# NingZhang1/pyscf_isdf

Measured on AMD Instinct MI355X. Metric: isdf_build_plus_get_jk_wall_time, lower is better.
Workload: dtype f64

## Files before the change

### include/mi355_isdf.h

```cpp
#ifndef MI355_ISDF_H
#define MI355_ISDF_H

#include <stdint.h>

#ifdef __cplusplus
extern "C" {
#endif

typedef struct isdf_ctx* isdf_handle;

#define ISDF_OK 0
#define ISDF_ERR_ARG 1
#define ISDF_ERR_HIP 2
#define ISDF_ERR_LIB 3
#define ISDF_ERR_NUM 4

int isdf_abi_version(void);

int isdf_create(int device_id, isdf_handle* out);
int isdf_destroy(isdf_handle h);
int isdf_set_stream(isdf_handle h, void* hip_stream);
const char* isdf_last_error(isdf_handle h);
int64_t isdf_workspace_bytes(isdf_handle h);
int isdf_release_workspace(isdf_handle h);
// ... 44 lines not shown
                   int nblk, const int64_t* blk_off, const int32_t* nip,
                   double tol, double tie_rtol,
                   double* d_L, int64_t ldL, int64_t* d_piv, int32_t* rank);

int isdf_select_ip_ws(isdf_handle h, const double* d_ao, int nao, int64_t ld,
                      int nblk, const int64_t* blk_off, const int32_t* nip,
                      double tol, double tie_rtol,
                      double* d_L, int64_t ldL, int64_t* d_piv, int32_t* rank,
                      void* d_work, int64_t work_bytes);
int64_t isdf_select_ip_work_bytes(int nao, int64_t m);

int isdf_select_ip_gram(isdf_handle h, double* d_A, int m, int64_t ldA, int nip, double tol, double tie_rtol,
                        int panel, int64_t* d_piv, int32_t* rank);

int isdf_select_ip_cplx(isdf_handle h, const double* d_ao, int nao, int nh, int64_t ld,
                        int nblk, const int64_t* blk_off, const int32_t* nip,
                        double tol, double tie_rtol,
                        double* d_L, int64_t ldL, int64_t* d_piv, int32_t* rank);

int isdf_fit_from_chol(isdf_handle h, double* d_L, int k, int64_t m, int64_t ldL,
                       const int64_t* d_piv);

int isdf_fit_prepare(isdf_handle h, const double* d_ao, int nao, int64_t ld,
                     const int64_t* d_ip, int P, double reg_rel, double* d_aoP, double* d_chol,
                     double* reg_used);
int isdf_fit_apply(isdf_handle h, const double* d_chol, const double* d_aoP, int P, int nao,
                   const double* d_ao, int64_t ng, int64_t ld, int forward_only,
                   double* d_theta, int64_t ldt);
int isdf_fit_prepare_cplx(isdf_handle h, const double* d_ao, int nao, int nh, int64_t ld,
                          const int64_t* d_ip, int P, double reg_rel, double* d_aoP, double* d_chol,
                          double* reg_used);
int isdf_fit_apply_cplx(isdf_handle h, const double* d_chol, const double* d_aoP, int P, int nao, int nh,
                        const double* d_ao, int64_t ng, int64_t ld, int forward_only,
                        double* d_theta, int64_t ldt);
int isdf_fit_global(isdf_handle h, const double* d_ao, int nao, int64_t ngrids, int64_t ld,
                    const int64_t* d_ip, int P, double reg_rel, double* d_theta, int64_t ldt,
                    double* d_aoP, double* reg_used);

int isdf_gather_aoP(isdf_handle h, const double* d_ao, int nao, int64_t ld, const int64_t* d_ip, int P,
                    double* d_aoP);
int isdf_gram_sq(isdf_handle h, const double* d_aoP, int P, int nao, int nh, double* d_A);
int isdf_pair_gram_rows(isdf_handle h, const double* d_aoP, int P, int nao, int nh, const double* d_ao,
                        int64_t ng, int64_t ld, double* d_B, int64_t ldb);
int isdf_block_chol(isdf_handle h, const double* d_A, int P, int nblk, const int32_t* blk_off,
                    double shift_rel, double* d_D, double* shift_used);
int isdf_block_solve(isdf_handle h, const double* d_D, int P, int nblk, const int32_t* blk_off, int side,
                     int trans, double* d_X, int64_t n, int64_t ldx);
int isdf_block_invert(isdf_handle h, const double* d_D, int P, int nblk, const int32_t* blk_off, double* d_Dinv);
int isdf_block_apply(isdf_handle h, const double* d_Dinv, int64_t ldd, int nblk, const int32_t* blk_off,
                     double* d_X, int64_t n, int64_t ldx);
int isdf_pair_rows_block_apply(isdf_handle h, const double* d_aoP, int P, int nao, const double* d_ao, int64_t ng,
                               int64_t ld, const double* d_Dinv, int64_t ldd, int nblk, const int32_t* blk_off,
                               double* d_B, int64_t ldb);

int isdf_gram_prod(isdf_handle h, const double* d_aoP, int P, int nao, const double* d_psiP, int nocc, double* d_A);
int isdf_pair_prod_rows(isdf_handle h, const double* d_aoP, int P, int nao, const double* d_psiP, int nocc,
                        const double* d_ao, int64_t ld, const double* d_psi, int64_t ldpsi, int64_t ng,
                        double* d_B, int64_t ldb);
int isdf_factor_solve_half(isdf_handle h, const double* d_fac, int P, int backward, double* d_X, int64_t n, int64_t ldx);
int isdf_gram_prod_cplx(isdf_handle h, const double* d_aoP, int P, int nao, int nh, const double* d_psiP, int npsi, int npsi_h,
                        double* d_A);
int isdf_pair_prod_rows_cplx(isdf_handle h, const double* d_aoP, int P, int nao, int nh, const double* d_psiP, int npsi,
                             int npsi_h, const double* d_ao, int64_t ld, const double* d_psi, int64_t ldpsi, int64_t ng,
                             double* d_B, int64_t ldb);

int isdf_shift_diag(isdf_handle h, double* d_A, int P, double shift_rel);
int isdf_chol_inplace(isdf_handle h, double* d_A, int P, double shift_rel, double* d_scratch, double* reg_used);

int isdf_factor_solve(isdf_handle h, const double* d_fac, int P, double* d_X, int64_t n, int64_t ldx);

int isdf_bj_probe_vectors(isdf_handle h, double* d_T, int n, const double* d_fac, const double* d_D, int P,
                          int nblk, const int32_t* blk_off);
int isdf_rows_combine(isdf_handle h, const double* d_E, int n, int64_t ldE, int rows, const double* d_Y,
                      int64_t ng, int64_t ldy, double* d_F, int64_t ldf, int accumulate);

int isdf_bj_probe_rows(isdf_handle h, double* d_T, int n, const double* d_fac, const double* d_D, int P, int nblk,
                       const int32_t* blk_off, const double* d_Yp, int64_t ng, int64_t ldy, double* d_F, int64_t ldf);

int isdf_gather_T(isdf_handle h, const double* d_L, int k, int64_t ldL, const int64_t* d_piv,
                  double* d_T);
int isdf_W_from_factor(isdf_handle h, const double* d_F, int P, int kind, double* d_M, int64_t ldm);

int isdf_coulomb_W(isdf_handle h, const double* d_theta, int P, int64_t ldt,
                   const int32_t mesh[3], const double a[9],
                   int row0, int nrows, int batch, int upper_only, double* d_W, int64_t ldw);
int isdf_coulG_half(isdf_handle h, const int32_t mesh[3], const double a[9], double* d_out);
int isdf_spectral_supported(isdf_handle h, const int32_t mesh[3], int batch, int* ok);
int isdf_spectral_rows(isdf_handle h, const double* d_in, int nrows, int64_t ld, const int32_t mesh[3], const int32_t* d_idx,
                       const double* d_scale, int npts, int batch, double* d_out, int64_t ldx);
int isdf_coulomb_rows(isdf_handle h, const double* d_in, int nrows, int64_t ld,
                      const int32_t mesh[3], const double a[9], int batch, double* d_out, int64_t ldo);
int isdf_symmetrize_upper(isdf_handle h, double* d_W, int P, int64_t ldw);
int isdf_symmetrize_mean(isdf_handle h, double* d_W, int P, int64_t ldw, int antisymmetric);

int isdf_get_j(isdf_handle h, const double* d_ao, int nao, int64_t ngrids, int64_t ld,
               const int32_t mesh[3], const double a[9],
               const double* d_dm, int nset, double* d_vj);
int isdf_rho(isdf_handle h, const double* d_ao, int nao, int64_t ng, int64_t ld,
             const double* d_dm, int nset, double* d_rho, int64_t ldrho);
int isdf_coulomb_potential(isdf_handle h, double* d_rho_inout, int nset, int64_t ldrho,
                           const int32_t mesh[3], const double a[9]);
int isdf_vj_from_vR(isdf_handle h, const double* d_ao, int nao, int64_t ng, int64_t ld,
                    const double* d_vR, int nset, int64_t ldv, double* d_vj);

int isdf_get_k_exact(isdf_handle h, const double* d_ao, int nao, int64_t ngrids, int64_t ld,
                     const double* d_C, int nocc, const int32_t mesh[3], const double a[9],
// ... 84 lines not shown
```

### pyscf_isdf_amd/backend.py

```python
import ctypes
import os
import numpy as np
import torch
from . import lib as _lib

_vp = ctypes.c_void_p


def _np_ptr(a):
    return a.ctypes.data_as(_vp)


class HipBackend:
    name = 'hip-gfx950'

    def __init__(self, device=0):
        if not torch.cuda.is_available():
            raise _lib.IsdfError('no GPU visible to torch; the ISDF path has no CPU fallback')
        self.device = torch.device('cuda', device)
        torch.cuda.set_device(self.device)
        self.handle = _lib.Handle(device)
        if os.environ.get('ISDF_TRSM') == 'subst':
            self.set_option('trsm_substitution', 1)
        if os.environ.get('ISDF_OWN_FFT') in ('0', '1', '2'):
# ... 232 lines not shown
    def gram_prod_cplx(self, aoP, nh, psiP, npsi_h, A):
        self._stream()
        assert aoP.is_contiguous() and psiP.is_contiguous() and A.is_contiguous() and aoP.shape[0] == psiP.shape[0]
        self.handle.call('isdf_gram_prod_cplx', self._p(aoP), aoP.shape[0], aoP.shape[1], int(nh), self._p(psiP), psiP.shape[1],
                         int(npsi_h), self._p(A))

    def pair_prod_rows_cplx(self, aoP, nh, psiP, npsi_h, ao, psi, ng, B):
        self._stream()
        assert aoP.is_contiguous() and psiP.is_contiguous() and aoP.shape[0] == psiP.shape[0]
        assert ao.stride(1) == 1 and psi.stride(1) == 1 and B.stride(1) == 1
        self.handle.call('isdf_pair_prod_rows_cplx', self._p(aoP), aoP.shape[0], aoP.shape[1], int(nh), self._p(psiP),
                         psiP.shape[1], int(npsi_h), self._p(ao), ao.stride(0), self._p(psi), psi.stride(0), int(ng), self._p(B),
                         B.stride(0))

    def factor_solve_half(self, fac, backward, X):
        self._stream()
        self.handle.call('isdf_factor_solve_half', self._p(fac), fac.shape[0], int(bool(backward)), self._p(X), X.shape[1],
                         X.stride(0))

    def block_chol(self, A, blk_off, shift_rel, D):
        self._stream()
        blk_off = np.ascontiguousarray(blk_off, dtype=np.int32)
        used = ctypes.c_double(0.0)
        self.handle.call('isdf_block_chol', self._p(A), A.shape[0], len(blk_off) - 1, _np_ptr(blk_off), float(shift_rel),
                         self._p(D), ctypes.byref(used))
        return used.value

    def block_solve(self, D, blk_off, side, trans, X):
        self._stream()
        blk_off = np.ascontiguousarray(blk_off, dtype=np.int32)
        n = X.shape[1] if side == 0 else X.shape[0]
        self.handle.call('isdf_block_solve', self._p(D), D.stride(0), len(blk_off) - 1, _np_ptr(blk_off), int(side), int(trans),
                         self._p(X), int(n), X.stride(0))

    def block_invert(self, D, blk_off, Dinv):
        self._stream()
        blk_off = np.ascontiguousarray(blk_off, dtype=np.int32)
        assert D.is_contiguous() and Dinv.is_contiguous() and Dinv.shape == D.shape
        self.handle.call('isdf_block_invert', self._p(D), D.shape[0], len(blk_off) - 1, _np_ptr(blk_off), self._p(Dinv))

    def block_apply(self, Dinv, blk_off, X):
        self._stream()
        blk_off = np.ascontiguousarray(blk_off, dtype=np.int32)
        self.handle.call('isdf_block_apply', self._p(Dinv), Dinv.stride(0), len(blk_off) - 1, _np_ptr(blk_off), self._p(X),
                         X.shape[1], X.stride(0))

    def pair_rows_block_apply(self, aoP, ao, ng, Dinv, blk_off, B):
        self._stream()
        blk_off = np.ascontiguousarray(blk_off, dtype=np.int32)
        assert aoP.stride(1) == 1 and aoP.stride(0) == aoP.shape[1]
        self.handle.call('isdf_pair_rows_block_apply', self._p(aoP), aoP.shape[0], aoP.shape[1], self._p(ao), int(ng), ao.stride(0),
                         self._p(Dinv), Dinv.stride(0), len(blk_off) - 1, _np_ptr(blk_off), self._p(B), B.stride(0))

    def shift_diag(self, A, shift_rel):
        self._stream()
        self.handle.call('isdf_shift_diag', self._p(A), A.shape[0], float(shift_rel))

    def chol_inplace(self, A, shift_rel, scratch=None):
        self._stream()
        reg = ctypes.c_double(0.0)
        assert scratch is None or scratch.numel() >= A.numel()
        self.handle.call('isdf_chol_inplace', self._p(A), A.shape[0], float(shift_rel),
                         self._p(scratch) if scratch is not None else None, ctypes.byref(reg))
        return reg.value

    def factor_solve(self, fac, X):
        self._stream()
        self.handle.call('isdf_factor_solve', self._p(fac), fac.shape[0], self._p(X), X.shape[1], X.stride(0))

    def bj_probe_rows(self, T, fac, D, blk_off, Yp, ng, F):
        self._stream()
        blk_off = np.ascontiguousarray(blk_off, dtype=np.int32)
        self.handle.call('isdf_bj_probe_rows', self._p(T), T.shape[0], self._p(fac), self._p(D), D.shape[0],
                         len(blk_off) - 1, _np_ptr(blk_off), self._p(Yp), int(ng), Yp.stride(0), self._p(F), F.stride(0))

    def bj_probe_vectors(self, T, fac, D, blk_off):
        self._stream()
        blk_off = np.ascontiguousarray(blk_off, dtype=np.int32)
        assert T.is_contiguous()
        self.handle.call('isdf_bj_probe_vectors', self._p(T), T.shape[0], self._p(fac), self._p(D), D.shape[0],
                         len(blk_off) - 1, _np_ptr(blk_off))

    def rows_combine(self, E, Y, F, accumulate=False):
        self._stream()
        assert E.stride(1) == 1 and Y.stride(1) == 1 and F.stride(1) == 1 and E.shape[1] == Y.shape[0]
        self.handle.call('isdf_rows_combine', self._p(E), E.shape[0], E.stride(0), E.shape[1], self._p(Y), Y.shape[1],
                         Y.stride(0), self._p(F), F.stride(0), int(bool(accumulate)))

    def gather_T(self, L, k, piv, T):
        self._stream()
        assert T.is_contiguous() and T.shape == (k, k)
        self.handle.call('isdf_gather_T', self._p(L), int(k), L.stride(0), self._p(piv), self._p(T))

    def W_from_factor(self, F, kind, M):
        self._stream()
        assert F.is_contiguous()
        self.handle.call('isdf_W_from_factor', self._p(F), M.shape[0], int(kind), self._p(M), M.stride(0))

    def fit_global(self, ao, ngrids, ip, reg_rel, theta, aoP):
        self._stream()
        assert ip.dtype == torch.int64 and aoP.is_contiguous()
        reg = ctypes.c_double(0.0)
        self.handle.call('isdf_fit_global', self._p(ao), ao.shape[0], int(ngrids), ao.stride(0), self._p(ip),
                         ip.numel(), float(reg_rel), self._p(theta), theta.stride(0), self._p(aoP), ctypes.byref(reg))
        return reg.value

# ... 361 lines not shown
```

### pyscf_isdf_amd/csrc/fit.hip

```cpp
#include "common.h"
#include <cstdlib>

namespace {

__global__ void gather_T_kernel(const double* __restrict__ L, int64_t ldL,
                                const int64_t* __restrict__ piv, int k, double* __restrict__ T) {
  const int s = blockIdx.x * blockDim.x + threadIdx.x;
  const int t = blockIdx.y;
  if (s >= k) return;
  T[(int64_t)t * k + s] = (s >= t) ? L[(int64_t)t * ldL + piv[s]] : 0.0;
}

__global__ void square_kernel(double* __restrict__ x, int64_t rows, int64_t cols, int64_t ld) {
  const int64_t c = (int64_t)blockIdx.x * blockDim.x + threadIdx.x;
  const int64_t r = blockIdx.y;
  if (c >= cols) return;
  const double v = x[r * ld + c];
  x[r * ld + c] = v * v;
}

__global__ void square_add_kernel(double* __restrict__ x, int64_t ld, const double* __restrict__ y, int64_t ldy,
                                  int64_t cols) {
  const int64_t c = (int64_t)blockIdx.x * blockDim.x + threadIdx.x;
  const int64_t r = blockIdx.y;
// ... 344 lines not shown
  ARG_CHECK(h, d_D && d_X && blk_off && P > 0 && nblk > 0 && n > 0 && (side == 0 || side == 1) && (trans == 0 || trans == 1));
  ARG_CHECK(h, n < 2147483647LL && ldx < 2147483647LL);
  if (side == 0 && trans == 0 && !h->trsm_substitution) {
    ARG_CHECK(h, blk_off[0] == 0 && blk_off[nblk] <= P);
    return block_forward_solve(h, d_D, P, nblk, blk_off, d_X, ldx, n);
  }
  for (int b = 0; b < nblk; ++b) {
    const int off = blk_off[b], nb = blk_off[b + 1] - off;
    if (nb <= 0) continue;
    const double* Db = d_D + (int64_t)off * P + off;
    const int rc = (side == 0) ? tri_left(h, trans != 0, nb, n, Db, P, d_X + (int64_t)off * ldx, ldx)
                               : tri_right(h, trans != 0, nb, n, Db, P, d_X + off, ldx);
    if (rc) return rc;
  }
  return ISDF_OK;
}

namespace {
__global__ void block_identity_kernel(double* __restrict__ E, int P, const int32_t* __restrict__ blk_of_row) {
  const int64_t i = (int64_t)blockIdx.x * blockDim.x + threadIdx.x;
  if (i < (int64_t)P * P) E[i] = (i / P == i % P) ? 1.0 : 0.0;
  (void)blk_of_row;
}
}

extern "C" int isdf_block_invert(isdf_handle h, const double* d_D, int P, int nblk, const int32_t* blk_off, double* d_Dinv) {
  if (!h) return ISDF_ERR_ARG;
  ARG_CHECK(h, d_D && d_Dinv && blk_off && P > 0 && nblk > 0 && blk_off[0] == 0 && blk_off[nblk] <= P);
  hipLaunchKernelGGL(block_identity_kernel, dim3((unsigned)cdiv((int64_t)P * P, 256)), dim3(256), 0, h->stream, d_Dinv, P,
                     (const int32_t*)nullptr);
  KERNEL_CHECK(h);
  return block_forward_solve(h, d_D, P, nblk, blk_off, d_Dinv, P, P);
}

extern "C" int isdf_block_apply(isdf_handle h, const double* d_Dinv, int64_t ldd, int nblk, const int32_t* blk_off,
                                double* d_X, int64_t n, int64_t ldx) {
  if (!h) return ISDF_ERR_ARG;
  ARG_CHECK(h, d_Dinv && d_X && blk_off && nblk > 0 && n > 0 && ldx >= n && blk_off[0] == 0 && blk_off[nblk] <= ldd);
  return block_apply_inverse(h, d_Dinv, ldd, nblk, blk_off, d_X, ldx, n);
}

extern "C" int isdf_pair_rows_block_apply(isdf_handle h, const double* d_aoP, int P, int nao, const double* d_ao, int64_t ng,
                                          int64_t ld, const double* d_Dinv, int64_t ldd, int nblk, const int32_t* blk_off,
                                          double* d_B, int64_t ldb) {
  if (!h) return ISDF_ERR_ARG;
  ARG_CHECK(h, d_aoP && d_ao && d_Dinv && d_B && blk_off && P > 0 && nao > 0 && ng > 0 && ld >= ng && ldb >= ng && nblk > 0);
  ARG_CHECK(h, blk_off[0] == 0 && blk_off[nblk] == P);
  const bool own = gemm_nn_f64_supported(h, P, ng, nao, d_aoP, nao, d_ao, ld);
  int rc = product_rows(h, P, ng, nao, d_aoP, d_ao, ld, d_B, ldb, own);
  if (rc) return rc;
  return block_apply_inverse(h, d_Dinv, ldd, nblk, blk_off, d_B, ldb, ng, !own);
}

extern "C" int isdf_shift_diag(isdf_handle h, double* d_A, int P, double shift_rel) {
  if (!h) return ISDF_ERR_ARG;
  ARG_CHECK(h, d_A && P > 0 && shift_rel >= 0);
  if (shift_rel == 0.0) return ISDF_OK;
  int* info = (int*)isdf_ws(h, "fit_info", 256);
  if (!info) return ISDF_ERR_HIP;
  double* maxdiag = (double*)(info + 16);
  hipLaunchKernelGGL(max_diag_kernel, dim3(1), dim3(256), 0, h->stream, d_A, P, maxdiag);
  hipLaunchKernelGGL(add_diag_kernel, dim3((unsigned)cdiv(P, 256)), dim3(256), 0, h->stream, d_A, P, maxdiag, shift_rel);
  KERNEL_CHECK(h);
  return ISDF_OK;
}

extern "C" int isdf_chol_inplace(isdf_handle h, double* d_A, int P, double shift_rel, double* d_scratch,
                                 double* reg_used) {
  if (!h) return ISDF_ERR_ARG;
  ARG_CHECK(h, d_A && P > 0 && shift_rel >= 0);
  int* info = (int*)isdf_ws(h, "fit_info", 256);
  double* keep = d_scratch ? d_scratch : (double*)isdf_ws(h, "chol_keep", sizeof(double) * (size_t)P * P);
  if (!info || !keep) return ISDF_ERR_HIP;
  double* maxdiag = (double*)(info + 16);
  HIP_TRY(h, hipMemcpyAsync(keep, d_A, sizeof(double) * (size_t)P * P, hipMemcpyDeviceToDevice, h->stream));
  double reg = shift_rel;
  for (int attempt = 0; attempt < 5; ++attempt) {
    if (attempt > 0)
      HIP_TRY(h, hipMemcpyAsync(d_A, keep, sizeof(double) * (size_t)P * P, hipMemcpyDeviceToDevice, h->stream));
    if (reg > 0) {
      hipLaunchKernelGGL(max_diag_kernel, dim3(1), dim3(256), 0, h->stream, d_A, P, maxdiag);
      hipLaunchKernelGGL(add_diag_kernel, dim3((unsigned)cdiv(P, 256)), dim3(256), 0, h->stream, d_A, P, maxdiag, reg);
      KERNEL_CHECK(h);
    }
    { ProfScope ps(h, "rocsolver_dpotrf[flop]", (double)P * P * P / 3.0);
      BLAS_TRY(h, rocsolver_dpotrf(h->blas, rocblas_fill_upper, P, d_A, P, info)); }
    int h_info = 0;
    HIP_TRY(h, hipMemcpyAsync(&h_info, info, sizeof(int), hipMemcpyDeviceToHost, h->stream));
    HIP_TRY(h, hipStreamSynchronize(h->stream));
    if (h_info == 0) {
      if (reg_used) *reg_used = reg;
      return ISDF_OK;
    }
    reg = (reg > 0.0) ? reg * 100.0 : 1e-14;
  }
  return isdf_fail(h, ISDF_ERR_NUM, "matrix is not numerically positive definite even with diagonal shift %g * max diag",
                   reg / 100.0);
}

extern "C" int isdf_factor_solve(isdf_handle h, const double* d_fac, int P, double* d_X, int64_t n, int64_t ldx) {
  if (!h) return ISDF_ERR_ARG;
  ARG_CHECK(h, d_fac && d_X && P > 0 && n > 0 && ldx >= n && n < 2147483647LL && ldx < 2147483647LL);
  int rc = tri_left(h, false, P, n, d_fac, P, d_X, ldx);
  if (rc) return rc;
  return tri_left(h, true, P, n, d_fac, P, d_X, ldx);
}
// ... 211 lines not shown
```

### pyscf_isdf_amd/fit_route.py

```python
import numpy as np


class FitRouteMixin:
    def _bj_prepare(self, ao, nh, d_ip, ip_off, aoP, scratch=None):
        be = self.backend
        P = aoP.shape[0]
        be.gather_aoP(ao, d_ip, aoP)
        A = self._buffer('factor', (P, P))
        if getattr(self, '_psi', None) is not None and not nh:
            be.gram_prod(aoP, self._psiP, A)
        else:
            be.gram_sq(aoP, A, nh)
        self._Dinv_key = None
        be.shift_diag(A, self.reg_rel)
        Dblk = self._buffer('Dblk', (P, P))
        self.block_shift_used = be.block_chol(A, ip_off, self.block_shift, Dblk)
        be.block_solve(Dblk, ip_off, 0, 0, A)
        be.block_solve(Dblk, ip_off, 1, 1, A)
        extra = be.chol_inplace(A, 0.0, scratch=scratch)
        self.reg_used = self.reg_rel + extra
        return A, Dblk

    def _block_inverse(self, Dblk, ip_off):
        if not self.block_apply_mfma or int(np.diff(np.asarray(ip_off)).max()) > 1100:
# ... 205 lines not shown

    def _sphere_energy_share(self, mesh, cg, mult, box, keep, w, ntest=8):
        import torch
        be = self.backend
        ao = getattr(self, 'ao', None)
        if ao is None:
            return np.inf
        nao, G = ao.shape
        rng = np.random.default_rng(7)
        cd = be.to_device(rng.standard_normal((2 * ntest, nao)) / np.sqrt(nao))
        rows = be.empty((2 * ntest, G))
        be.gemm_nn(cd, ao, rows)
        t = rows[:ntest].contiguous()
        be.hadamard_rows(t, rows[ntest:].contiguous())
        Gfull = int(np.prod(mesh))
        if G != Gfull:
            g0, g1 = self._slice
            full = be.zeros((ntest, Gfull))
            full[:, g0:g1] = t
            self.comm.all_reduce_sum(full)
            t = full
        idx = np.flatnonzero(box.ravel()).astype(np.int32)
        scale = np.sqrt(mult.ravel()[idx] * w * cg.ravel()[idx])
        ldx = -(-2 * len(idx) // 128) * 128
        X = be.empty((ntest, ldx))
        be.spectral_rows(t, mesh, be.to_device(idx), be.to_device(scale), X, batch=ntest)
        x = be.to_host(X)[:, :2 * len(idx)]
        e = x[:, 0::2] ** 2 + x[:, 1::2] ** 2
        outside = ~keep.ravel()[idx]
        tot = e.sum(axis=1)
        return float((e[:, outside].sum(axis=1) / np.where(tot > 0, tot, 1.0)).max())

    def _finish_W_spectral(self, W, probe=None):
        be, st = self.backend, self._fit_state
        plan = self._spectral_plan()
        ip_off = np.asarray(st['ip_off'], dtype=np.int64)
        P = W.shape[0]
        mesh = np.asarray(self.mesh, dtype=np.int32)
        G = int(np.prod(mesh))
        if plan is None:
            rows_avail = int(self._bufs['theta'].numel() // G)
            st2 = dict(st, kind='blockjacobi-paneled', rows=self._buffer('theta', (rows_avail, G)),
                       panels=self._panel_plan(ip_off, rows_avail))
            self._fit_state = st2
            try:
                return self._finish_W_paneled(W, probe=probe)
            finally:
                self._fit_state = st
        nbat = int(self.fft_batch or 512)
        big = int(np.diff(ip_off).max())
        self._last_fft_batch = nbat
        ldx = plan['ldx']
        X = self._buffer('theta', (P, ldx))
        scratch = self._buffer('rows_scratch', (nbat + big, G))
        self.w_spectral_fraction = plan['fraction']
        self._last_spectral_ldx = ldx
        nxt, fill, g0 = 0, 0, 0
        while nxt < P or fill > 0:
            while fill < nbat and nxt < P:
                i = int(np.searchsorted(ip_off, nxt))
                j = i + 1
                while j + 1 < len(ip_off) and fill + (ip_off[j + 1] - nxt) <= nbat + big:
                    j += 1
                b1 = int(ip_off[j])
                self._bj_rows_range(nxt, b1, scratch[fill:fill + (b1 - nxt)])
                fill += b1 - nxt
                nxt = b1
            take = min(nbat, fill)
            rows = scratch[:take]
            if probe is not None:
                be.rows_combine(probe[0][:, g0:g0 + take], rows, probe[1], accumulate=g0 > 0)
            be.spectral_rows(rows, mesh, plan['idx'], plan['scale'], X[g0:g0 + take], batch=take)
            if fill > take:
                scratch[:fill - take].copy_(scratch[take:fill].clone() if fill - take > take else scratch[take:fill])
            g0 += take
            fill -= take
        for b0 in range(0, P, nbat):
            b1 = min(P, b0 + nbat)
            be.gemm_nt(X[b0:b1], X[b0:], W[b0:b1, b0:], alpha=1.0)
        be.symmetrize_upper(W)
        self._bj_finish(st['Afac'], st['Dblk'], st['ip_off'], W)

    def _bj_finish(self, Afac, Dblk, ip_off, W, antisymmetric=False):
        be = self.backend
        be.W_from_factor(Afac, 2, W)
        be.W_from_factor(Afac, 0, W)
        be.block_solve(Dblk, ip_off, 0, 1, W)
        be.block_solve(Dblk, ip_off, 1, 0, W)
        be.symmetrize_mean(W, antisymmetric)

    def _bj_clusters(self):
        cell = self.cell
        natm = cell.natm
        parent = list(range(natm))

        def find(i):
            while parent[i] != i:
                parent[i] = parent[parent[i]]
                i = parent[i]
            return i
        r = float(self.bj_cluster_radius or 0.0)
        if r > 0 and natm > 1:
            a = np.asarray(cell.lattice_vectors(), dtype=float)
            frac = np.asarray(cell.atom_coords(), dtype=float).dot(np.linalg.inv(a))
            d = frac[:, None, :] - frac[None, :, :]
            d -= np.round(d)
            dist = np.linalg.norm(d.dot(a), axis=2)
            for i, j in zip(*np.nonzero(np.triu(dist < r, 1))):
                ri, rj = find(int(i)), find(int(j))
                if ri != rj:
                    parent[max(ri, rj)] = min(ri, rj)
        groups = {}
        for i in range(natm):
            groups.setdefault(find(i), []).append(i)
        return [groups[k] for k in sorted(groups)]

    def _bj_blocks(self, counts, clusters):
        per = [int(sum(counts[b] for b in cl)) for cl in clusters]
        off = np.append(0, np.cumsum(per)).astype(np.int32)
        g = max(1, int(self.bj_group))
        if g > 1:
            off = np.unique(np.append(off[::g], off[-1])).astype(np.int32)
        return off

    def _fit_routes(self):
        if self.fit_route not in ('auto', 'blockjacobi', 'cholesky'):
            raise ValueError("fit_route must be 'auto', 'blockjacobi' or 'cholesky'")
        if self._want_theta or self.fit_route == 'cholesky':
            return ['cholesky']
        if self.fit_route == 'blockjacobi':
            return ['blockjacobi']
        if self.c_isdf > self.bj_max_c:
            return ['cholesky']
        return ['blockjacobi', 'cholesky']
# ... 80 lines not shown
```

### pyscf_isdf_amd/isdf.py

```python
import os
import sys
import time
import warnings
import numpy as np
import torch
from . import gto
from ._common import (UniformGrids, partition_grid_by_atom, _monkhorst_pack_size, _aoslice_by_atom,
                      _default_fft_batch)
from .fit_route import FitRouteMixin
from .sharded import ShardedMixin
from .kpoints import KPointMixin
from .hcore import HcoreMixin
from .eri_surface import EriSurfaceMixin


class ISDF(FitRouteMixin, ShardedMixin, KPointMixin, HcoreMixin, EriSurfaceMixin):
    _keys = {'cell', 'kpts', 'grids', 'mesh', 'blockdim', 'exxdiv', 'c_isdf', 'select', 'tie_rtol'}

    def __init__(self, cell, kpts=np.zeros((1, 3)), c_isdf=12, select='refined', backend=None, comm=None):
        self.cell = cell
        self.stdout = getattr(cell, 'stdout', None) or sys.stdout
        self.verbose = getattr(cell, 'verbose', 0)
        self.max_memory = getattr(cell, 'max_memory', 4000)
        self.kpts_symm = None
        if hasattr(kpts, 'kpts_ibz') and hasattr(kpts, 'transform_dm'):
            self.kpts_symm = kpts
            kpts = kpts.kpts
        self.kpts = np.asarray(kpts).reshape(-1, 3)
        self.grids = UniformGrids(cell, cell.mesh)
        self.blockdim = 240
        self.exxdiv = None
        self.c_isdf = c_isdf
        self.select = select
        self.refine_over = 2.0
        self.pair_space = 'ao'
        self.occ_refit = 'always'
        self.w_spectral = True
        self.w_sphere = 'auto'
        self.w_sphere_tol = 1e-11
        self.w_sort_bins = 256
        self.w_spectral_check_tol = 5e-9
        self.w_spectral_max_c = 18
        self.cand_skip_zero_rows = True
        self.cand_gram = True
        self.cand_ao_cutoff = None
        self.tie_rtol = 1e-10
        self.select_tol = -1.0
        self.reg_rel = 1e-12
        self.reg_used = 0.0
        self.k_ip_factor = None
        self.kpt_pair_q = 'auto'
        self.kpt_w_spectral = False
        self.kpts_band = None
        self.force_sharded = False
        self.fit_route = 'auto'
        self.bj_check_tol = 3e-8
        self.bj_auto_kpts = False
        self.bj_max_c = 12
        self.bj_nprobe = 8
        self.bj_cluster_radius = 2.4
        self.bj_group = 1
        self.bj_check = None
        self.fit_route_used = None
        self.block_shift = 0.0
        self.block_shift_used = 0.0
        self.robust_k = False
        self.explicit_theta = False
        self.fft_batch = None
        self.block_apply_mfma = True
        self.max_resident_rows = None
        self.max_device_memory = None
        self.n_panels = 1
        self._backend = backend
        self._comm = comm
        self._rsh_df = {}
        self._built = False
        self._W_omega = {}
        self._fit_state = None
        self._fit_pending = False
        self._psi = self._psiP = None
        self._fit_dm = None
        self._V = None
        self._bufs = {}
        self._ovlp = None
        self.timings = {}
        self.ao = None
        self.aoP = None
        self.W = None
        self.ip = None

    @property
    def _want_theta(self):
        return bool(self.explicit_theta or self.robust_k)

    @property
    def _sharded(self):
        return self.comm.size > 1 or self.force_sharded or getattr(self.comm, 'always', False)

    @property
    def mesh(self):
        return self.grids.mesh

    @mesh.setter
    def mesh(self, mesh):
        self.grids.mesh = np.asarray(mesh)
        self.grids._coords = None

    @property
    def backend(self):
        if self._backend is None:
            from .backend import HipBackend
            dev = 0
            if self._comm is not None:
                dev = self._comm.local_rank
            if os.environ.get('ISDF_ONE_GPU'):
                dev = 0
            self._backend = HipBackend(dev)
        return self._backend

    def reset(self, cell=None):
        if cell is not None:
# ... 876 lines not shown
```

### pyscf_isdf_amd/lib.py

```python
import ctypes
import os

_HERE = os.path.dirname(os.path.abspath(__file__))
LIB_PATH = os.path.join(_HERE, 'lib', 'libmi355_isdf.so')
ABI_VERSION = 21

_lib = None

c_int, c_i64, c_dbl, c_vp = ctypes.c_int, ctypes.c_int64, ctypes.c_double, ctypes.c_void_p

SIGNATURES = {
    'isdf_abi_version': (c_int, []),
    'isdf_create': (c_int, [c_int, ctypes.POINTER(c_vp)]),
    'isdf_destroy': (c_int, [c_vp]),
    'isdf_set_stream': (c_int, [c_vp, c_vp]),
    'isdf_last_error': (ctypes.c_char_p, [c_vp]),
    'isdf_workspace_bytes': (c_i64, [c_vp]),
    'isdf_set_coulomb_omega': (c_int, [c_vp, c_dbl]),
    'isdf_set_coulomb_cutoff': (c_int, [c_vp, c_dbl]),
    'isdf_set_coulomb_ws': (c_int, [c_vp, c_dbl, c_vp, c_vp, c_vp, c_vp]),
    'isdf_set_option': (c_int, [c_vp, ctypes.c_char_p, c_int]),
    'isdf_release_workspace': (c_int, [c_vp]),
    'isdf_prof_enable': (c_int, [c_vp, c_int]),
    'isdf_prof_reset': (c_int, [c_vp]),
    'isdf_prof_count': (c_int, [c_vp]),
    'isdf_prof_get': (c_int, [c_vp, c_int, ctypes.c_char_p, c_int, ctypes.POINTER(c_i64), ctypes.POINTER(c_dbl), ctypes.POINTER(c_dbl)]),
    'isdf_eval_ao': (c_int, [c_vp, c_vp, c_int, c_vp, c_int, c_vp, c_int, c_vp, c_int, c_vp, c_vp, c_i64, c_vp, c_i64]),
    'isdf_block_row_absmax': (c_int, [c_vp, c_vp, c_int, c_i64, c_int, c_vp, c_vp]),
    'isdf_gather_cols': (c_int, [c_vp, c_vp, c_int, c_i64, c_vp, c_i64, c_vp, c_i64]),
    'isdf_partition_by_atom': (c_int, [c_vp, c_vp, c_i64, c_vp, c_int, c_vp, c_dbl, c_vp]),
    'isdf_select_ip': (c_int, [c_vp, c_vp, c_int, c_i64, c_int, c_vp, c_vp, c_dbl, c_dbl, c_vp, c_i64, c_vp, c_vp]),
    'isdf_select_ip_ws': (c_int, [c_vp, c_vp, c_int, c_i64, c_int, c_vp, c_vp, c_dbl, c_dbl, c_vp, c_i64, c_vp, c_vp, c_vp,
                                  c_i64]),
    'isdf_select_ip_work_bytes': (c_i64, [c_int, c_i64]),
    'isdf_select_ip_gram': (c_int, [c_vp, c_vp, c_int, c_i64, c_int, c_dbl, c_dbl, c_int, c_vp, ctypes.POINTER(ctypes.c_int32)]),
    'isdf_fit_from_chol': (c_int, [c_vp, c_vp, c_int, c_i64, c_i64, c_vp]),
    'isdf_fit_prepare': (c_int, [c_vp, c_vp, c_int, c_i64, c_vp, c_int, c_dbl, c_vp, c_vp, ctypes.POINTER(c_dbl)]),
    'isdf_fit_apply': (c_int, [c_vp, c_vp, c_vp, c_int, c_int, c_vp, c_i64, c_i64, c_int, c_vp, c_i64]),
    'isdf_gather_aoP': (c_int, [c_vp, c_vp, c_int, c_i64, c_vp, c_int, c_vp]),
    'isdf_gram_sq': (c_int, [c_vp, c_vp, c_int, c_int, c_int, c_vp]),
    'isdf_pair_gram_rows': (c_int, [c_vp, c_vp, c_int, c_int, c_int, c_vp, c_i64, c_i64, c_vp, c_i64]),
    'isdf_gram_prod': (c_int, [c_vp, c_vp, c_int, c_int, c_vp, c_int, c_vp]),
    'isdf_pair_prod_rows': (c_int, [c_vp, c_vp, c_int, c_int, c_vp, c_int, c_vp, c_i64, c_vp, c_i64, c_i64, c_vp, c_i64]),
    'isdf_factor_solve_half': (c_int, [c_vp, c_vp, c_int, c_int, c_vp, c_i64, c_i64]),
    'isdf_gram_prod_cplx': (c_int, [c_vp, c_vp, c_int, c_int, c_int, c_vp, c_int, c_int, c_vp]),
    'isdf_pair_prod_rows_cplx': (c_int, [c_vp, c_vp, c_int, c_int, c_int, c_vp, c_int, c_int, c_vp, c_i64, c_vp, c_i64, c_i64,
                                         c_vp, c_i64]),
    'isdf_block_chol': (c_int, [c_vp, c_vp, c_int, c_int, c_vp, c_dbl, c_vp, ctypes.POINTER(c_dbl)]),
    'isdf_block_solve': (c_int, [c_vp, c_vp, c_int, c_int, c_vp, c_int, c_int, c_vp, c_i64, c_i64]),
    'isdf_block_invert': (c_int, [c_vp, c_vp, c_int, c_int, c_vp, c_vp]),
    'isdf_block_apply': (c_int, [c_vp, c_vp, c_i64, c_int, c_vp, c_vp, c_i64, c_i64]),
    'isdf_pair_rows_block_apply': (c_int, [c_vp, c_vp, c_int, c_int, c_vp, c_i64, c_i64, c_vp, c_i64, c_int, c_vp, c_vp, c_i64]),
    'isdf_shift_diag': (c_int, [c_vp, c_vp, c_int, c_dbl]),
    'isdf_chol_inplace': (c_int, [c_vp, c_vp, c_int, c_dbl, c_vp, ctypes.POINTER(c_dbl)]),
    'isdf_factor_solve': (c_int, [c_vp, c_vp, c_int, c_vp, c_i64, c_i64]),
    'isdf_bj_probe_vectors': (c_int, [c_vp, c_vp, c_int, c_vp, c_vp, c_int, c_int, c_vp]),
    'isdf_rows_combine': (c_int, [c_vp, c_vp, c_int, c_i64, c_int, c_vp, c_i64, c_i64, c_vp, c_i64, c_int]),
    'isdf_bj_probe_rows': (c_int, [c_vp, c_vp, c_int, c_vp, c_vp, c_int, c_int, c_vp, c_vp, c_i64, c_i64, c_vp, c_i64]),
    'isdf_gather_T': (c_int, [c_vp, c_vp, c_int, c_i64, c_vp, c_vp]),
    'isdf_W_from_factor': (c_int, [c_vp, c_vp, c_int, c_int, c_vp, c_i64]),
    'isdf_fit_global': (c_int, [c_vp, c_vp, c_int, c_i64, c_i64, c_vp, c_int, c_dbl, c_vp, c_i64, c_vp, ctypes.POINTER(c_dbl)]),
    'isdf_coulomb_W': (c_int, [c_vp, c_vp, c_int, c_i64, c_vp, c_vp, c_int, c_int, c_int, c_int, c_vp, c_i64]),
    'isdf_coulomb_rows': (c_int, [c_vp, c_vp, c_int, c_i64, c_vp, c_vp, c_int, c_vp, c_i64]),
    'isdf_symmetrize_upper': (c_int, [c_vp, c_vp, c_int, c_i64]),
    'isdf_symmetrize_mean': (c_int, [c_vp, c_vp, c_int, c_i64, c_int]),
    'isdf_get_j': (c_int, [c_vp, c_vp, c_int, c_i64, c_i64, c_vp, c_vp, c_vp, c_int, c_vp]),
    'isdf_rho': (c_int, [c_vp, c_vp, c_int, c_i64, c_i64, c_vp, c_int, c_vp, c_i64]),
    'isdf_coulomb_potential': (c_int, [c_vp, c_vp, c_int, c_i64, c_vp, c_vp]),
    'isdf_vj_from_vR': (c_int, [c_vp, c_vp, c_int, c_i64, c_i64, c_vp, c_int, c_i64, c_vp]),
    'isdf_eval_ao_k': (c_int, [c_vp, c_vp, c_int, c_vp, c_int, c_vp, c_int, c_vp, c_int, c_vp, c_vp, c_int, c_vp, c_i64, c_vp, c_vp, c_i64]),
    'isdf_select_ip_cplx': (c_int, [c_vp, c_vp, c_int, c_int, c_i64, c_int, c_vp, c_vp, c_dbl, c_dbl, c_vp, c_i64, c_vp, c_vp]),
    'isdf_fit_prepare_cplx': (c_int, [c_vp, c_vp, c_int, c_int, c_i64, c_vp, c_int, c_dbl, c_vp, c_vp, ctypes.POINTER(c_dbl)]),
    'isdf_fit_apply_cplx': (c_int, [c_vp, c_vp, c_vp, c_int, c_int, c_int, c_vp, c_i64, c_i64, c_int, c_vp, c_i64]),
    'isdf_coulG_q': (c_int, [c_vp, c_vp, c_vp, c_vp, c_int, c_dbl, c_vp]),
    'isdf_coulomb_Wq': (c_int, [c_vp, c_vp, c_int, c_i64, c_vp, c_vp, c_dbl, c_int, c_int, c_int, c_int, c_vp, c_vp, c_i64]),
    'isdf_symmetrize_hermitian': (c_int, [c_vp, c_vp, c_vp, c_int, c_i64]),
    'isdf_finish_Wq': (c_int, [c_vp, c_vp, c_vp, c_int, c_i64, c_vp, c_vp]),
    'isdf_get_k_pair': (c_int, [c_vp, c_vp, c_vp, c_vp, c_vp, c_int, c_int, c_dbl, c_vp]),
    'isdf_get_k_exact_kpt': (c_int, [c_vp, c_vp, c_vp, c_int, c_i64, c_vp, c_vp, c_int, c_i64, c_vp, c_vp, c_dbl, c_int, c_int, c_int, c_vp, c_vp]),
    'isdf_coulG_half': (c_int, [c_vp, c_vp, c_vp, c_vp]),
    'isdf_spectral_supported': (c_int, [c_vp, c_vp, c_int, ctypes.POINTER(c_int)]),
    'isdf_spectral_rows': (c_int, [c_vp, c_vp, c_int, c_i64, c_vp, c_vp, c_vp, c_int, c_int, c_vp, c_i64]),
    'isdf_coulomb_rows_q': (c_int, [c_vp, c_vp, c_int, c_i64, c_vp, c_vp, c_vp, c_vp]),
    'isdf_nyquist_spectra': (c_int, [c_vp, c_vp, c_int, c_i64, c_vp, c_int, c_vp, c_vp]),
    'isdf_zhadamard_planes': (c_int, [c_vp, c_vp, c_vp, c_i64, c_vp, c_vp, c_i64, c_int, c_i64]),
    'isdf_rho_k': (c_int, [c_vp, c_vp, c_vp, c_int, c_i64, c_i64, c_vp, c_vp, c_dbl, c_vp]),
    'isdf_vj_k': (c_int, [c_vp, c_vp, c_vp, c_int, c_i64, c_i64, c_vp, c_vp, c_vp]),
    'isdf_pp_local_potential': (c_int, [c_vp, c_int, c_vp, c_vp, c_vp, c_vp, c_vp]),
    'isdf_pp_projector_overlaps': (c_int, [c_vp, c_vp, c_int, c_vp, c_int, c_vp, c_int, c_vp, c_vp, c_vp, c_vp, c_int, c_vp, c_vp, c_vp]),
    'isdf_gemm_nn': (c_int, [c_vp, c_int, c_i64, c_int, c_dbl, c_vp, c_i64, c_vp, c_i64, c_dbl, c_vp, c_i64]),
    'isdf_hadamard_rows': (c_int, [c_vp, c_vp, c_i64, c_vp, c_i64, c_int, c_i64]),
    'isdf_eval_ao_deriv1': (c_int, [c_vp, c_vp, c_int, c_vp, c_int, c_vp, c_int, c_vp, c_int, c_vp, c_vp, c_i64, c_vp, c_i64, c_i64]),
    'isdf_eval_ao_k_deriv1': (c_int, [c_vp, c_vp, c_int, c_vp, c_int, c_vp, c_int, c_vp, c_int, c_vp, c_vp, c_int, c_vp, c_i64, c_vp, c_vp, c_i64, c_i64]),
    'isdf_uniform_grid': (c_int, [c_vp, c_vp, c_vp, c_vp]),
    'isdf_rho_pair': (c_int, [c_vp, c_vp, c_int, c_vp, c_int, c_i64, c_i64, c_vp, c_int, c_vp, c_i64]),
    'isdf_mg_embed_density': (c_int, [c_vp, c_vp, c_int, c_vp, c_dbl, c_vp, c_vp, c_int]),
    'isdf_mg_restrict_potential': (c_int, [c_vp, c_vp, c_int, c_vp, c_vp, c_dbl, c_vp]),
    'isdf_mg_coulomb_kernel': (c_int, [c_vp, c_vp, c_int, c_vp, c_vp]),
    'isdf_lda_exchange': (c_int, [c_vp, c_vp, c_i64, c_vp, c_vp]),
    'isdf_lda_vwn_add': (c_int, [c_vp, c_vp, c_i64, c_vp, c_vp]),
    'isdf_gga_b88': (c_int, [c_vp, c_vp, c_vp, c_i64, c_i64, c_vp, c_vp, c_vp, c_i64]),
    'isdf_xc_fused': (c_int, [c_vp, c_vp, c_vp, c_i64, c_i64, c_dbl, c_dbl, c_dbl, c_int, c_dbl, c_vp, c_vp, c_vp, c_i64]),
    'isdf_gga_lyp_polarised': (c_int, [c_vp, c_vp, c_vp, c_i64, c_i64, c_i64, c_dbl, c_int, c_vp, c_vp, c_vp, c_i64, c_i64]),
    'isdf_lda_exchange_fxc': (c_int, [c_vp, c_vp, c_i64, c_vp]),
    'isdf_lda_vwn_fxc_add': (c_int, [c_vp, c_vp, c_i64, c_vp]),
# ... 67 lines not shown
```

Baseline: 16.92.

## Stream pair rows through aligned frontiers, applying block inverse only to completed blocks

Adds a two-frontier schedule for the spectral W build. Pair-product rows are produced in aligned pieces, and the block-diagonal inverse is applied only up to the last fully produced block boundary, after which the spectral transform runs. Leftover rows carry over to the next piece. This replaces per-batch calls with larger, aligned GEMM and inverse-apply launches, which should use the matrix units better and cut repeated work, at the cost of more host-side bookkeeping and a scratch copy of the tail rows.

```diff
diff --git a/include/mi355_isdf.h b/include/mi355_isdf.h
--- a/include/mi355_isdf.h
+++ b/include/mi355_isdf.h
@@ -120,6 +120,11 @@
 int isdf_pair_rows_block_apply(isdf_handle h, const double* d_aoP, int P, int nao, const double* d_ao, int64_t ng,
                                int64_t ld, const double* d_Dinv, int64_t ldd, int nblk, const int32_t* blk_off,
                                double* d_B, int64_t ldb);
+int isdf_pair_rows_squared(isdf_handle h, const double* d_aoP, int rows, int nao, const double* d_ao, int64_t ng,
+                           int64_t ld, int* squared);
+int isdf_pair_rows_frontier(isdf_handle h, const double* d_aoP, int nnew, int nao, const double* d_ao, int64_t ng,
+                            int64_t ld, int squared, const double* d_Dinv, int64_t ldd, int nblk, const int32_t* blk_off,
+                            double* d_B, int64_t ldb, int have);
 
 int isdf_gram_prod(isdf_handle h, const double* d_aoP, int P, int nao, const double* d_psiP, int nocc, double* d_A);
 int isdf_pair_prod_rows(isdf_handle h, const double* d_aoP, int P, int nao, const double* d_psiP, int nocc,
diff --git a/pyscf_isdf_amd/backend.py b/pyscf_isdf_amd/backend.py
--- a/pyscf_isdf_amd/backend.py
+++ b/pyscf_isdf_amd/backend.py
@@ -308,6 +308,24 @@
         self.handle.call('isdf_pair_rows_block_apply', self._p(aoP), aoP.shape[0], aoP.shape[1], self._p(ao), int(ng), ao.stride(0),
                          self._p(Dinv), Dinv.stride(0), len(blk_off) - 1, _np_ptr(blk_off), self._p(B), B.stride(0))
 
+    def pair_rows_squared(self, aoP, rows, ao, ng):
+        self._stream()
+        sq = ctypes.c_int(0)
+        self.handle.call('isdf_pair_rows_squared', self._p(aoP), int(rows), aoP.shape[1], self._p(ao), int(ng), ao.stride(0),
+                         ctypes.byref(sq))
+        return bool(sq.value)
+
+    def pair_rows_frontier(self, aoP_new, ao, ng, squared, Dinv, blk_off, B, have):
+        self._stream()
+        blk_off = np.ascontiguousarray(blk_off, dtype=np.int32)
+        nnew = aoP_new.shape[0]
+        assert aoP_new.stride(1) == 1 and aoP_new.stride(0) == aoP_new.shape[1] and B.stride(1) == 1
+        assert have + nnew <= B.shape[0] and blk_off[0] == 0 and blk_off[-1] <= have + nnew and B.shape[1] >= ng
+        assert len(blk_off) == 1 or (Dinv.shape[0] >= blk_off[-1] and Dinv.shape[1] >= blk_off[-1])
+        self.handle.call('isdf_pair_rows_frontier', self._p(aoP_new) if nnew else None, nnew, aoP_new.shape[1], self._p(ao), int(ng),
+                         ao.stride(0), int(bool(squared)), self._p(Dinv) if len(blk_off) > 1 else None, Dinv.stride(0) if len(blk_off) > 1 else 0,
+                         len(blk_off) - 1, _np_ptr(blk_off), self._p(B), B.stride(0), int(have))
+
     def shift_diag(self, A, shift_rel):
         self._stream()
         self.handle.call('isdf_shift_diag', self._p(A), A.shape[0], float(shift_rel))
diff --git a/pyscf_isdf_amd/csrc/fit.hip b/pyscf_isdf_amd/csrc/fit.hip
--- a/pyscf_isdf_amd/csrc/fit.hip
+++ b/pyscf_isdf_amd/csrc/fit.hip
@@ -420,6 +420,30 @@
   return block_apply_inverse(h, d_Dinv, ldd, nblk, blk_off, d_B, ldb, ng, !own);
 }
 
+extern "C" int isdf_pair_rows_squared(isdf_handle h, const double* d_aoP, int rows, int nao, const double* d_ao, int64_t ng,
+                                      int64_t ld, int* squared) {
+  if (!h) return ISDF_ERR_ARG;
+  ARG_CHECK(h, d_aoP && d_ao && squared && rows > 0 && nao > 0 && ng > 0 && ld >= ng);
+  *squared = gemm_nn_f64_supported(h, rows, ng, nao, d_aoP, nao, d_ao, ld) ? 1 : 0;
+  return ISDF_OK;
+}
+
+extern "C" int isdf_pair_rows_frontier(isdf_handle h, const double* d_aoP, int nnew, int nao, const double* d_ao, int64_t ng,
+                                       int64_t ld, int squared, const double* d_Dinv, int64_t ldd, int nblk,
+                                       const int32_t* blk_off, double* d_B, int64_t ldb, int have) {
+  if (!h) return ISDF_ERR_ARG;
+  ARG_CHECK(h, d_ao && d_B && nnew >= 0 && nnew <= 65535 && have >= 0 && nblk >= 0 && nao > 0 && ng > 0 && ld >= ng && ldb >= ng);
+  ARG_CHECK(h, (nnew == 0 || d_aoP) && (nblk == 0 || (d_Dinv && blk_off && blk_off[0] == 0 && blk_off[nblk] <= have + nnew)));
+  if (nnew > 0) {
+    double* rows = d_B + (int64_t)have * ldb;
+    int rc = squared ? product_rows(h, nnew, ng, nao, d_aoP, d_ao, ld, rows, ldb, true)
+                     : gemm_rm(h, 'N', 'N', nnew, ng, nao, 1.0, d_aoP, nao, d_ao, ld, 0.0, rows, ldb);
+    if (rc) return rc;
+  }
+  if (nblk == 0) return ISDF_OK;
+  return block_apply_inverse(h, d_Dinv, ldd, nblk, blk_off, d_B, ldb, ng, !squared);
+}
+
 extern "C" int isdf_shift_diag(isdf_handle h, double* d_A, int P, double shift_rel) {
   if (!h) return ISDF_ERR_ARG;
   ARG_CHECK(h, d_A && P > 0 && shift_rel >= 0);
diff --git a/pyscf_isdf_amd/fit_route.py b/pyscf_isdf_amd/fit_route.py
--- a/pyscf_isdf_amd/fit_route.py
+++ b/pyscf_isdf_amd/fit_route.py
@@ -281,9 +281,13 @@
         self._last_fft_batch = nbat
         ldx = plan['ldx']
         X = self._buffer('theta', (P, ldx))
+        piece = self._pair_rows_piece(big)
         scratch = self._buffer('rows_scratch', (nbat + big, G))
         self.w_spectral_fraction = plan['fraction']
         self._last_spectral_ldx = ldx
+        if piece:
+            self._spectral_rows_two_frontiers(X, scratch, piece, plan, probe)
+            return self._spectral_W_finish(X, W, nbat)
         nxt, fill, g0 = 0, 0, 0
         while nxt < P or fill > 0:
             while fill < nbat and nxt < P:
@@ -304,11 +308,52 @@
                 scratch[:fill - take].copy_(scratch[take:fill].clone() if fill - take > take else scratch[take:fill])
             g0 += take
             fill -= take
+        self._spectral_W_finish(X, W, nbat)
+
+    def _spectral_W_finish(self, X, W, nbat):
+        be, st = self.backend, self._fit_state
+        P = W.shape[0]
         for b0 in range(0, P, nbat):
             b1 = min(P, b0 + nbat)
             be.gemm_nt(X[b0:b1], X[b0:], W[b0:b1, b0:], alpha=1.0)
         be.symmetrize_upper(W)
         self._bj_finish(st['Afac'], st['Dblk'], st['ip_off'], W)
+
+    def _pair_rows_piece(self, big):
+        align = int(getattr(self, 'pair_rows_align', 0) or 0)
+        if align <= 0 or not hasattr(self.backend, 'pair_rows_frontier') or getattr(self, '_psi', None) is not None \
+                or not self.block_apply_mfma or big > 1100:
+            return 0
+        return int(self.fft_batch or 512) // align * align
+
+    def _spectral_rows_two_frontiers(self, X, scratch, piece, plan, probe):
+        be, st = self.backend, self._fit_state
+        ip_off = np.asarray(st['ip_off'], dtype=np.int64)
+        P = int(ip_off[-1])
+        mesh = np.asarray(self.mesh, dtype=np.int32)
+        G = self.ao.shape[1]
+        Dinv = self._block_inverse(st['Dblk'], ip_off)
+        nbat = int(self.fft_batch or 512)
+        squared = be.pair_rows_squared(self.aoP, min(piece, P), self.ao, G)
+        app, prod = 0, 0
+        while app < P:
+            new = min(piece, P - prod)
+            j = int(np.searchsorted(ip_off, prod + new, side='right')) - 1
+            i = int(np.searchsorted(ip_off, app))
+            end = int(ip_off[j])
+            be.pair_rows_frontier(self.aoP[prod:prod + new], self.ao, G, squared, Dinv[app:, app:],
+                                  (ip_off[i:j + 1] - app).astype(np.int32), scratch, prod - app)
+            prod += new
+            if end > app:
+                rows = scratch[:end - app]
+                if probe is not None:
+                    be.rows_combine(probe[0][:, app:end], rows, probe[1], accumulate=app > 0)
+                be.spectral_rows(rows, mesh, plan['idx'], plan['scale'], X[app:end], batch=min(nbat, end - app))
+                tail = prod - end
+                if tail > 0:
+                    src = scratch[end - app:prod - app]
+                    scratch[:tail].copy_(src.clone() if tail > end - app else src)
+                app = end
 
     def _bj_finish(self, Afac, Dblk, ip_off, W, antisymmetric=False):
         be = self.backend
diff --git a/pyscf_isdf_amd/isdf.py b/pyscf_isdf_amd/isdf.py
--- a/pyscf_isdf_amd/isdf.py
+++ b/pyscf_isdf_amd/isdf.py
@@ -67,6 +67,7 @@
         self.robust_k = False
         self.explicit_theta = False
         self.fft_batch = None
+        self.pair_rows_align = 256
         self.block_apply_mfma = True
         self.max_resident_rows = None
         self.max_device_memory = None
diff --git a/pyscf_isdf_amd/lib.py b/pyscf_isdf_amd/lib.py
--- a/pyscf_isdf_amd/lib.py
+++ b/pyscf_isdf_amd/lib.py
@@ -51,6 +51,9 @@
     'isdf_block_invert': (c_int, [c_vp, c_vp, c_int, c_int, c_vp, c_vp]),
     'isdf_block_apply': (c_int, [c_vp, c_vp, c_i64, c_int, c_vp, c_vp, c_i64, c_i64]),
     'isdf_pair_rows_block_apply': (c_int, [c_vp, c_vp, c_int, c_int, c_vp, c_i64, c_i64, c_vp, c_i64, c_int, c_vp, c_vp, c_i64]),
+    'isdf_pair_rows_squared': (c_int, [c_vp, c_vp, c_int, c_int, c_vp, c_i64, c_i64, ctypes.POINTER(c_int)]),
+    'isdf_pair_rows_frontier': (c_int, [c_vp, c_vp, c_int, c_int, c_vp, c_i64, c_i64, c_int, c_vp, c_i64, c_int, c_vp, c_vp, c_i64,
+                                        c_int]),
     'isdf_shift_diag': (c_int, [c_vp, c_vp, c_int, c_dbl]),
     'isdf_chol_inplace': (c_int, [c_vp, c_vp, c_int, c_dbl, c_vp, ctypes.POINTER(c_dbl)]),
     'isdf_factor_solve': (c_int, [c_vp, c_vp, c_int, c_vp, c_i64, c_i64]),
```

Measured after the change: 16.68 (median of 6 runs). -1.4%, faster.
